# anneouyang/OuterSPACE

Measured on AMD Instinct MI355X. Metric: spgemm_output_nnz_per_s, higher is better.
Workload: dtype f64

## Files before the change

### outerspace_amd/csrc/osp_pipeline.h

```cpp
#pragma once

#define OSP_WITH_RA(ctx_, ...)                                               \
    do {                                                                     \
        if ((ctx_)->rank_atomic) { constexpr bool RA = true; __VA_ARGS__; }  \
        else { constexpr bool RA = false; __VA_ARGS__; }                     \
    } while (0)

template <class T> struct PanelWork {
    uint64_t r0, r1;
    bool whole;
    uint64_t base, count;
    Part<T> *stage;
    const uint32_t *cells = nullptr; Part<T> *qstage = nullptr;
    const HubArgs *hub = nullptr;
    bool compact = false;
    bool has_long = true;
    bool desc_only = false;
    bool walk_all = false;
};
template <class T> struct Producer {
    virtual ~Producer() {}
    virtual void produce(const PanelWork<T> &w, PhaseTimer &tm) = 0;
};

// ... 204 lines not shown
        fprintf(stderr, "[osp]   panel rows [%llu,%llu): %u tiles, %u long rows with %llu partial products -> %llu segments; direct: %llu rows, %llu "
                        "partial products, %llu cells\n",
                (unsigned long long)r0, (unsigned long long)r1, pl.p0.ntiles, nlong, (unsigned long long)pl.nh, (unsigned long long)pl.nvirt,
                (unsigned long long)pl.mode_rows[kModeDirect], (unsigned long long)pl.mode_partials[kModeDirect], (unsigned long long)ndcell);
    pl.ghist = sc.get<uint32_t>(pl.ncell + 1);
    pl.ghist_tmp = sc.get<uint32_t>(scan_scratch_entries(pl.ncell + 1));
    pl.vrow_off = sc.get<uint64_t>(pl.nvirt + 1);
    pl.vfirst = sc.get<uint8_t>(pl.nvirt + 1);
    pl.vcol0 = sc.get<uint32_t>(pl.nvirt + 1);
    pl.vcol1 = sc.get<uint32_t>(pl.nvirt + 1);
    if (pl.mode_rows[kModeDirect]) {
        pl.cells = sc.get<uint32_t>(ndcell);
        GatherPlan gp{};
        RunDesc<T> *runs = nullptr;
        const uint64_t max_runs = env.gather_max_runs.or_(0xffffffffull);
        if (ds->gather && nrund && nrd < max_runs) {
            runs = sc.get<RunDesc<T>>(std::max<uint64_t>(nrd, 1));
            pl.vrun_off = sc.get<uint32_t>(pl.nvirt + 1);
            pl.vrun_end = sc.get<uint32_t>(pl.nvirt + 1);
            gp.rdbase = rdbase; gp.vrun_off = pl.vrun_off; gp.vrun_end = pl.vrun_end;
            gp.rowruns = sc.get<uint32_t>(nlong);
            pl.nwritten = gp.nwritten = sc.get<uint32_t>(1);
            fill_async(s, {{pl.vrun_off, (pl.nvirt + 1) * sizeof(uint32_t), kNoRuns}, {gp.rowruns, (uint64_t)nlong * sizeof(uint32_t), kNoRuns},
                           {pl.nwritten, sizeof(uint32_t), 0u}});
            gp.over = env.gather_over.on;
            gp.av_in_order = ds->av_in_order ? 1u : 0u;
            pl.may_write = !gp.over;
            pl.ga.runs = runs; pl.ga.b_colidx = ds->b_colidx; pl.ga.b_vals = (const T *)ds->b_vals;
        }
        if (!(runs && gp.over) || (hub_b && pl.nblocks)) ds->ensure_chunk_off(s);
        gp.mark_skipped = ds->chunk_off_ready ? 1u : 0u;
        const bool plan_small = runs != nullptr && gp.over && nsmall != 0;
        const bool plan_big = !plan_small || nsmall < pl.mode_rows[kModeDirect];
        if (plan_small) gp.small = hsmall;
        if (ctx->env.verbose)
            fprintf(stderr, "[osp]   small planner: %llu of %llu direct rows (at most %u chunks, %u cells)\n", (unsigned long long)(plan_small ? nsmall : 0),
                    (unsigned long long)pl.mode_rows[kModeDirect], small_lim.chunks, small_lim.cells);
        tm.begin(PH_PLAN_K, s);
        if (plan_small)
            direct_plan_small_kernel<T><<<nlong, kWave, direct_plan_small_lds(small_lim.cells), s>>>(
                pl.p0.long_rows, nlong, pl.hbits, nseg, pl.vbase, pl.hoff, colbits, kCap, ds->rowfirst, ds->off, ds->bs, ds->perm, ds->b_colidx,
                pl.vrow_off, pl.vcol0, pl.vcol1, ds->chunk_off, gp, (const T *)ds->a_vals, runs);
        if (!plan_big) {  }
        else if (nlong <= 4u * ctx->cus)
            direct_plan_kernel<T, kDirectCellsBig><<<nlong, kDirectThreads, 0, s>>>(pl.p0.long_rows, nlong, pl.hmode, pl.hbits, nseg, pl.vbase, pl.hoff,
                                                                                 pl.cellbase, row_off, colbits, kCap, ds->rowfirst, ds->off, ds->bs, ds->perm,
                                                                                 ds->b_colidx, pl.vrow_off, pl.vcol0, pl.vcol1, pl.cells, ds->chunk_off, gp,
                                                                                 (const T *)ds->a_vals, runs);
        else
        direct_plan_kernel<T><<<nlong, kDirectThreads, 0, s>>>(pl.p0.long_rows, nlong, pl.hmode, pl.hbits, nseg, pl.vbase, pl.hoff, pl.cellbase, row_off,
                                                              colbits, kCap, ds->rowfirst, ds->off, ds->bs, ds->perm, ds->b_colidx, pl.vrow_off,
                                                              pl.vcol0, pl.vcol1, pl.cells, ds->chunk_off, gp, (const T *)ds->a_vals, runs);
        tm.end(PH_PLAN_K);
        if (gp.rowruns && ds->gstat) gather_stats_kernel<<<std::min(grid_for(nlong, 256), 64u), 256, 0, s>>>(pl.p0.long_rows, nlong, row_off, gp.rowruns, ds->gstat);
#ifdef OSP_PLAN_PROF
        if (ctx->env.verbose) {
            unsigned long long hp[8] = {0}, z[8] = {0};
            OSP_HIP(hipStreamSynchronize(s));
// ... 714 lines not shown
```

### outerspace_amd/csrc/osp_settings.h

```cpp
#pragma once
#include <cstdint>
#include <cstdlib>
#include <string>

namespace osp {

struct Flag {
    bool set = false;
    int value = 0;
    explicit operator bool() const { return set; }
    void parse(const char *v) { set = v != nullptr; value = v ? atoi(v) : 0; }
};
struct Switch {
    bool on = true;
    explicit operator bool() const { return on; }
    void parse(const char *v) { on = !(v && *v && atoi(v) == 0); }
};
template <class T> struct Opt {
    bool set = false;
    T value{};
    T or_(T dflt) const { return set ? value : dflt; }
};
struct Int : Opt<int> { void parse(const char *v) { if ((set = v && *v)) value = atoi(v); } };
struct Long : Opt<long> { void parse(const char *v) { if ((set = v && *v)) value = atol(v); } };
// ... 3 lines not shown
    std::string text;
    bool is(const char *w) const { return text == w; }
    void parse(const char *v) { text = v ? v : ""; }
};

enum When { PerCall, PerContext, PerProcess };

#define OSP_SETTINGS(X)                                                   \
    X(verbose, "OSP_VERBOSE", Flag, PerCall)                              \
    X(sync, "OSP_SYNC", Flag, PerProcess)                                 \
    X(poison, "OSP_POISON", Flag, PerProcess)                             \
    X(guard, "OSP_GUARD", Flag, PerProcess)                               \
    X(direct, "OSP_DIRECT", Switch, PerCall)                              \
    X(hub, "OSP_HUB", Switch, PerCall)                                    \
    X(plan_small, "OSP_PLAN_SMALL", Switch, PerCall)                      \
    X(gather_over, "OSP_GATHER_OVER", Switch, PerCall)                    \
    X(expand_rows, "OSP_EXPAND_ROWS", Switch, PerCall)                    \
    X(plan_overlap, "OSP_PLAN_OVERLAP", Switch, PerCall)                  \
    X(gather, "OSP_GATHER", Int, PerCall)                                 \
    X(split_from_b, "OSP_SPLIT_FROM_B", Int, PerCall)                     \
    X(dense_seg, "OSP_DENSE_SEG", Int, PerCall)                           \
    X(multi_subpanels, "OSP_MULTI_SUBPANELS", Int, PerCall)               \
    X(parse_threads, "OSP_PARSE_THREADS", Int, PerCall)                   \
    X(plan_small_cells, "OSP_PLAN_SMALL_CELLS", Long, PerCall)            \
    X(plan_small_chunks, "OSP_PLAN_SMALL_CHUNKS", Long, PerCall)          \
    X(direct_min_nnz, "OSP_DIRECT_MIN_NNZ", U64, PerCall)                 \
    X(direct_max, "OSP_DIRECT_MAX", U64, PerCall)                         \
    X(split_row_max, "OSP_SPLIT_ROW_MAX", U64, PerCall)                   \
    X(gather_max_runs, "OSP_GATHER_MAX_RUNS", U64, PerCall)               \
    X(bigtile_cap, "OSP_BIGTILE_CAP", U64, PerCall)                       \
    X(compact_min_waste, "OSP_COMPACT_MIN_WASTE", U64, PerCall)           \
    X(masked_heavy_min, "OSP_MASKED_HEAVY_MIN", U64, PerCall)             \
    X(masked_bucket, "OSP_MASKED_BUCKET", U64, PerCall)                   \
    X(mcl_long_min, "OSP_MCL_LONG_MIN", U64, PerCall)                     \
    X(mxm_short_cap, "OSP_MXM_SHORT_CAP", U64, PerCall)                   \
    X(mxm_batch, "OSP_MXM_BATCH", U64, PerCall)                           \
    X(mxv_group, "OSP_MXV_GROUP", U64, PerCall)                           \
    X(hub_min_share, "OSP_HUB_MIN_SHARE", Real, PerCall)                  \
    X(hub_min_run, "OSP_HUB_MIN_RUN", Real, PerCall)                      \
    X(rank, "OSP_RANK", Word, PerContext)                                 \
// ... 30 lines not shown
```

### outerspace_amd/csrc/osp_split.h

```cpp
#pragma once
#include "osp_kernels.h"

namespace osp {

#ifndef OSP_SPLIT_THREADS
#define OSP_SPLIT_THREADS 256
#endif
constexpr int kSplitThreads = OSP_SPLIT_THREADS;
#ifndef OSP_SPLIT_ROW_THREADS
#define OSP_SPLIT_ROW_THREADS 1024
#endif
#ifndef OSP_SPLIT_ROW_PRE
#define OSP_SPLIT_ROW_PRE 1
#endif
constexpr int kSplitRowThreads = OSP_SPLIT_ROW_THREADS;
#ifndef OSP_SPLIT_ROW_STRETCH
#define OSP_SPLIT_ROW_STRETCH 4096
#endif
constexpr int kSplitRowStretch = OSP_SPLIT_ROW_STRETCH;
#ifndef OSP_SPLIT_STRETCH
#define OSP_SPLIT_STRETCH 4096
#endif
constexpr int kSplitStretch = OSP_SPLIT_STRETCH;
#ifndef OSP_SPLIT_JOB_ROUNDS
// ... 553 lines not shown
    uint32_t *nwritten = nullptr;
    uint32_t over = 1;
    uint32_t mark_skipped = 1;
    uint32_t av_in_order = 0;
    const uint8_t *small = nullptr;
};
__global__ void gather_stats_kernel(const uint32_t *rows, uint32_t nlong, const uint64_t *row_off, const uint32_t *rowruns, unsigned long long *gstat) {
    uint64_t nr = 0, np = 0, nd = 0;
    for (uint32_t h = blockIdx.x * blockDim.x + threadIdx.x; h < nlong; h += gridDim.x * blockDim.x) {
        const uint32_t r = rowruns[h];
        if (r != kNoRuns) { nr++; nd += r; np += row_off[rows[h] + 1] - row_off[rows[h]]; }
    }
    nr = wave_reduce_sum<uint64_t>(nr); np = wave_reduce_sum<uint64_t>(np); nd = wave_reduce_sum<uint64_t>(nd);
    if (lane_id() == 0 && nr) { atomicAdd(&gstat[0], (unsigned long long)nr); atomicAdd(&gstat[1], (unsigned long long)np); atomicAdd(&gstat[2], (unsigned long long)nd); }
}
constexpr int kDirectCellsBig = 8 * OSP_DIRECT_CELLS_LDS;
template <class V, int CL = OSP_DIRECT_CELLS_LDS>
__global__ __launch_bounds__(kDirectThreads, (CL > OSP_DIRECT_CELLS_LDS ? 2 : 8)) void direct_plan_kernel(
    const uint32_t *__restrict__ rows, uint32_t nlong, const uint8_t *__restrict__ hmode, const uint8_t *__restrict__ hbits,
    const uint32_t *__restrict__ nseg, const uint64_t *__restrict__ vbase, const uint64_t *__restrict__ hoff,
    const uint64_t *__restrict__ cellbase, const uint64_t *__restrict__ row_off, int colbits, uint32_t cap,
    const uint32_t *__restrict__ rowfirst, const uint64_t *__restrict__ ct_off, const uint32_t *__restrict__ ct_bs,
    const uint32_t *__restrict__ perm, const uint32_t *__restrict__ b_colidx, uint64_t *__restrict__ vrow_off,
    uint32_t *__restrict__ vcol0, uint32_t *__restrict__ vcol1, uint32_t *__restrict__ cells, uint64_t *__restrict__ chunk_off,
    const GatherPlan gp, const V *__restrict__ a_vals, RunDesc<V> *__restrict__ runs) {
    constexpr int NT = kDirectThreads, NFINE = 1 << kDirectFineBits, CBL = kDirectChunkBlock, UNR = OSP_DIRECT_UNR;
    constexpr int kCellsLds = CL;
    constexpr bool kBigCells = CL > OSP_DIRECT_CELLS_LDS;
    __shared__ V avs_own[kBigCells ? CBL : 1];
    __shared__ alignas(8) uint32_t hist[NFINE + 1];
    __shared__ alignas(4) uint16_t nxt[NFINE];
    __shared__ uint8_t lut[NFINE];
    __shared__ uint32_t rbin0[kDirectMaxRanges + 2], roff[kDirectMaxRanges + 2], cursor[kDirectMaxRanges + 1];
    __shared__ uint32_t cbs[CBL], cst[CBL + 1];
    __shared__ uint32_t cellm[kCellsLds], lsm[kCellsLds];
    __shared__ uint32_t psum[NT];
    __shared__ uint32_t scratch[NT / kWave + 1];
    __shared__ uint32_t s_T, s_over;
    const uint32_t h = blockIdx.x;
    if (h >= nlong || hmode[h] != kModeDirect) return;
    if (gp.small != nullptr && gp.small[h]) return;
    OSP_PLAN_DECL
    const unsigned tid = threadIdx.x, lane = lane_id(), w = tid >> 6;
    const uint64_t above = lanes_above_mask();
    const uint32_t i = rows[h];
    const uint32_t c0 = rowfirst[i], nc = rowfirst[i + 1] - c0;
    const uint32_t b = hbits[h], nfine = 1u << b, Ta = nseg[h];
    const int sh = colbits - (int)b;
    const uint32_t q0 = (uint32_t)hoff[h];
    uint32_t *__restrict__ rb = cells + cellbase[h];
    const uint32_t lutw = (nfine + 3) / 4;
    auto load_block = [&](uint32_t cb, uint32_t nb) {
        uint32_t len[CBL / NT], bsv[CBL / NT], sum = 0;
#pragma unroll
        for (int q = 0; q < CBL / NT; q++) {
            const uint32_t j = tid * (CBL / NT) + q;
            len[q] = 0; bsv[q] = 0;
            if (j < nb) {
                const uint32_t c = c0 + cb + j;
                bsv[q] = ct_bs[c];
                len[q] = (uint32_t)(ct_off[c + 1] - ct_off[c]);
            }
            sum += len[q];
        }
        uint32_t total;
        uint32_t ex = block_excl_scan<uint32_t, NT>(sum, scratch, &total);
#pragma unroll
        for (int q = 0; q < CBL / NT; q++) {
            const uint32_t j = tid * (CBL / NT) + q;
            if (j < nb) { cst[j] = ex; cbs[j] = bsv[q] - ex; }
            ex += len[q];
        }
        if (tid == 0) cst[nb] = total;
        __syncthreads();
        return total;
    };
// ... 4 lines not shown
#pragma unroll
            for (int u = 0; u < UNR; u++) {
                const uint32_t e = base + u * kWave + lane;
                const bool valid = e < E;
                while (valid && e >= cst[c + 1]) c++;
                cu[u] = c;
                col[u] = b_colidx[valid ? cbs[c] + e : 0u];
            }
#pragma unroll
            for (int u = 0; u < UNR; u++) f(cu[u], col[u], base + u * kWave + lane < E);
        }
    };
    for (uint32_t d = tid; d <= nfine; d += NT) hist[d] = 0;
    __syncthreads();
    OSP_PLAN_MARK(0);
    uint32_t have_cb = 0, have_nb = 0, have_E = 0;
    for (uint32_t cb = 0; cb < nc; cb += CBL) {
        const uint32_t nb = min((uint32_t)CBL, nc - cb);
        const uint32_t E = load_block(cb, nb);
        OSP_PLAN_MARK(1);
        have_cb = cb; have_nb = nb; have_E = E;
        for_entries(nb, E, [&](uint32_t, uint32_t col, bool valid) {
#if OSP_PLAN_RUNS
            const uint32_t bin = valid ? col >> sh : 0xffffffffu;
            uint32_t runlen;
            if (wave_run_head(bin, valid, runlen, above)) atomicAdd(&hist[bin], runlen);
#else
            if (valid) atomicAdd(&hist[col >> sh], 1u);
#endif
        });
        __syncthreads();
        OSP_PLAN_MARK(2);
    }
    {
        constexpr int PER = NFINE / NT;
        static_assert(NFINE % NT == 0 && PER >= 1, "the fine bins are scanned PER per thread");
        uint32_t v[PER], sum = 0;
#pragma unroll
        for (int q = 0; q < PER; q++) { const uint32_t d = tid * PER + q; v[q] = d < nfine ? hist[d] : 0u; sum += v[q]; }
        uint32_t total;
        uint32_t ex = block_excl_scan<uint32_t, NT>(sum, scratch, &total);
#pragma unroll
        for (int q = 0; q < PER; q++) { const uint32_t d = tid * PER + q; if (d < nfine) hist[d] = ex; ex += v[q]; }
        if (tid == 0) hist[nfine] = total;
    }
    __syncthreads();
    for (uint32_t d = tid; d < nfine; d += NT) {
        const uint32_t lim = hist[d] + cap;
// ... 32 lines not shown
        const bool multi = nc > CB;
        V *avs = kBigCells ? avs_own : reinterpret_cast<V *>(hist);
        uint32_t *nzc = reinterpret_cast<uint32_t *>(nxt), *ncur = rbin0;
        static_assert(sizeof(nxt) >= (kDirectMaxRanges + 1) * sizeof(uint32_t), "runs per range: where the grouping's chain was");
        const uint32_t rowbase = (uint32_t)gp.rdbase[h];
        static_assert(kDirectMaxRanges + 1 <= NT, "one range per thread");
        const uint32_t bcol_t = tid <= T ? (uint32_t)min((uint64_t)rbin0[tid] << sh, (uint64_t)0xffffffffu) : 0u;
        __syncthreads();
        if (tid <= T) { nzc[tid] = 0; ncur[tid] = 0; if (tid < T) cursor[tid] = bcol_t; }
        if (!multi) { for (uint32_t cl = tid; cl < nc; cl += NT) avs[cl] = gp.av_in_order ? a_vals[c0 + cl] : a_vals[perm[c0 + cl]]; }
        __syncthreads();
        for (uint32_t cb = 0; cb < nc; cb += CB) {
            const uint32_t nb = min(CB, nc - cb);
            for (uint32_t x = tid; x < nb * T; x += NT) cellm[x] = 0;
            uint32_t E = have_E;
            if (cb != have_cb || nb != have_nb) E = load_block(cb, nb);
            else __syncthreads();
            have_cb = cb; have_nb = nb; have_E = E;
            OSP_PLAN_MARK(1);
            if (T > 1 && (uint64_t)E >= (uint64_t)nb * (T - 1) * 8u) {
                for (uint32_t x = tid; x < nb * (T - 1); x += NT) {
                    const uint32_t cl = x / (T - 1), t = x - cl * (T - 1) + 1;
                    const uint32_t col = cursor[t], b0 = cbs[cl] + cst[cl];
                    uint32_t lo = 0, hi = cst[cl + 1] - cst[cl];
                    while (lo < hi) { const uint32_t mid = (lo + hi) >> 1; if (b_colidx[b0 + mid] < col) lo = mid + 1; else hi = mid; }
                    lsm[cl * T + t] = lo;
                }
                for (uint32_t cl = tid; cl < nb; cl += NT) lsm[cl * T] = 0;
                __syncthreads();
                for (uint32_t x = tid; x < nb * T; x += NT) {
                    const uint32_t cl = x / T, t = x - cl * T;
// ... 3 lines not shown
                for_entries(nb, E, [&](uint32_t cl, uint32_t col, bool valid) {
                    const uint32_t key = valid ? __umul24(cl, T) + (uint32_t)lut[col >> sh] : 0xffffffffu;
                    uint32_t runlen;
                    if (wave_run_head(key, valid, runlen, above)) atomicAdd(&cellm[key], runlen);
                });
            }
            __syncthreads();
            OSP_PLAN_MARK(4);
            for (uint32_t x = tid; x < nb * T; x += NT) {
                const uint32_t c = cellm[x], cl = x / T, t = x - cl * T;
                if (c) atomicAdd(&nzc[t], 1u);
                if (multi) rb[lutw + (uint64_t)(cb + cl) * Ta + t] = c;
            }
            __syncthreads();
        }
        {
            const uint32_t v = tid < T ? nzc[tid] : 0u;
            uint32_t total;
            const uint32_t ex = block_excl_scan<uint32_t, NT>(v, scratch, &total);
            if (tid < T) nzc[tid] = ex;
            if (tid == 0) {
                nzc[T] = total;
                gp.rowruns[h] = total;
            }
            if (tid < T) cursor[tid] = 0;
        }
        __syncthreads();
        for (uint32_t t = tid; t < Ta; t += NT) {
            const uint64_t v = vbase[h] + t;
            gp.vrun_off[v] = rowbase + nzc[min(t, T)];
            gp.vrun_end[v] = rowbase + nzc[min(t + 1, T)];
        }
        const uint32_t G = max(1u, min((uint32_t)NT / T, 16u));
        for (uint32_t cb = 0; cb < nc; cb += CB) {
            const uint32_t nb = min(CB, nc - cb);
            if (multi) {
                if (cb != have_cb || nb != have_nb) { have_E = load_block(cb, nb); have_cb = cb; have_nb = nb; }
                for (uint32_t x = tid; x < nb * T; x += NT) { const uint32_t cl = x / T, t = x - cl * T; cellm[x] = rb[lutw + (uint64_t)(cb + cl) * Ta + t]; }
            }
            if (multi) { for (uint32_t cl = tid; cl < nb; cl += NT) avs[cl] = gp.av_in_order ? a_vals[c0 + cb + cl] : a_vals[perm[c0 + cb + cl]]; }
            __syncthreads();
            for (uint32_t cl = tid; cl < nb; cl += NT) {
                uint32_t run = 0;
                for (uint32_t t = 0; t < T; t++) { lsm[cl * T + t] = run; run += cellm[cl * T + t]; }
            }
            const uint32_t S = (nb + G - 1) / G;
            for (uint32_t t0 = 0; t0 < T; t0 += NT) {
                const uint32_t Tb = min((uint32_t)NT, T - t0);
                const uint32_t g = tid / Tb, t = t0 + (tid - g * Tb);
                const bool on = g < G;
                uint32_t run0 = 0, nrun0 = 0;
                __syncthreads();
// ... 28 lines not shown
            if (gp.mark_skipped) { for (uint32_t cl = tid; cl < nb; cl += NT) chunk_off[perm[c0 + cb + cl]] = kChunkSkip; }
            __syncthreads();
            OSP_PLAN_MARK(5);
        }
        return;
    }
    for (uint32_t d = tid; d < lutw * 4; d += NT) reinterpret_cast<uint8_t *>(rb)[d] = d < nfine ? lut[d] : (uint8_t)0;
    if (tid == 0 && gp.rdbase != nullptr && gp.nwritten) atomicAdd(gp.nwritten, 1u);
    OSP_PLAN_MARK(3);
    const uint32_t CB = max(1u, min((uint32_t)CBL, (uint32_t)kCellsLds / T));
    const uint32_t G = max(1u, min((uint32_t)NT / T, 16u));
    for (uint32_t cb = 0; cb < nc; cb += CB) {
        const uint32_t nb = min(CB, nc - cb);
        for (uint32_t x = tid; x < nb * T; x += NT) cellm[x] = 0;
        uint32_t E = have_E;
        if (cb != have_cb || nb != have_nb) E = load_block(cb, nb);
        else __syncthreads();
        have_cb = cb; have_nb = nb; have_E = E;
        OSP_PLAN_MARK(1);
        for_entries(nb, E, [&](uint32_t cl, uint32_t col, bool valid) {
#if OSP_PLAN_RUNS
            const uint32_t key = valid ? __umul24(cl, T) + (uint32_t)lut[col >> sh] : 0xffffffffu;
            uint32_t runlen;
            if (wave_run_head(key, valid, runlen, above)) atomicAdd(&cellm[key], runlen);
#else
            if (valid) atomicAdd(&cellm[__umul24(cl, T) + (uint32_t)lut[col >> sh]], 1u);
#endif
        });
        __syncthreads();
        OSP_PLAN_MARK(4);
        for (uint32_t cl = tid; cl < nb; cl += NT) {
// ... 18 lines not shown
                uint32_t run = run0;
                for (uint32_t gg = 0; gg < g; gg++) run += psum[gg * Tb + (t - t0)];
                const uint32_t rbase = q0 + roff[t];
                for (uint32_t cl = g * S; cl < min(nb, (g + 1) * S); cl++) {
                    rb[lutw + (uint64_t)(cb + cl) * Ta + t] = rbase + run - lsm[cl * T + t];
                    run += cellm[cl * T + t];
                }
                if (g == G - 1) cursor[t] = run;
            }
        }
        for (uint32_t cl = tid; cl < nb; cl += NT)
            chunk_off[perm[c0 + cb + cl]] = direct_desc((uint32_t)cellbase[h], lutw + (cb + cl) * Ta, (uint32_t)sh);
        __syncthreads();
        OSP_PLAN_MARK(5);
    }
}
__device__ __forceinline__ void wave_lds_sync() {
    __builtin_amdgcn_fence(__ATOMIC_RELEASE, "wavefront");
    __builtin_amdgcn_wave_barrier();
    __builtin_amdgcn_fence(__ATOMIC_ACQUIRE, "wavefront");
}
__device__ __forceinline__ uint32_t wave_last(uint32_t v) { return (uint32_t)__builtin_amdgcn_readlane((int)v, kWave - 1); }
constexpr size_t direct_plan_small_lds(uint32_t cells) { return (size_t)cells * sizeof(uint32_t); }
template <class V>
__global__ __launch_bounds__(kWave, 8) void direct_plan_small_kernel(
    const uint32_t *__restrict__ rows, uint32_t nlong, const uint8_t *__restrict__ hbits, const uint32_t *__restrict__ nseg,
    const uint64_t *__restrict__ vbase, const uint64_t *__restrict__ hoff, int colbits, uint32_t cap,
    const uint32_t *__restrict__ rowfirst, const uint64_t *__restrict__ ct_off, const uint32_t *__restrict__ ct_bs,
    const uint32_t *__restrict__ perm, const uint32_t *__restrict__ b_colidx, uint64_t *__restrict__ vrow_off,
    uint32_t *__restrict__ vcol0, uint32_t *__restrict__ vcol1, uint64_t *__restrict__ chunk_off, const GatherPlan gp,
    const V *__restrict__ a_vals, RunDesc<V> *__restrict__ runs) {
    constexpr int NF = 1 << kSmallFineBits, UNR = OSP_DIRECT_UNR, RMAX = kSmallRanges;
    extern __shared__ uint32_t cell[];
    __shared__ alignas(8) uint32_t hist[NF + 2];
    __shared__ uint32_t psum[kWave];
    __shared__ uint32_t cbs[kWave], cst[kWave + 1];
    __shared__ uint32_t rbin0[RMAX + 1], roff[RMAX + 1], bcol[RMAX + 1], nzc[RMAX + 1];
    static_assert(sizeof(hist) >= kSmallChunks * sizeof(V), "the A values go where the histogram was");
    static_assert(kSmallChunks <= kWave && kSmallRanges <= kWave && kSmallCellsMin >= NF, "a lane per chunk, a lane per segment, the chain in the cells");
    const uint32_t h = blockIdx.x;
    if (h >= nlong || !gp.small[h]) return;
    OSP_PLAN_DECL
    const unsigned lane = lane_id();
    const uint64_t above = lanes_above_mask();
    const uint32_t i = rows[h];
    const uint32_t c0 = rowfirst[i], nc = rowfirst[i + 1] - c0;
    const uint32_t b = hbits[h], nfine = 1u << b, Ta = nseg[h];
    const int sh = colbits - (int)b;
    const uint32_t q0 = (uint32_t)hoff[h];
    uint32_t bs = 0, len = 0, pa = 0;
    if (lane < nc) {
        const uint32_t c = c0 + lane;
        bs = ct_bs[c];
        len = (uint32_t)(ct_off[c + 1] - ct_off[c]);
        pa = perm[c];
    }
    const V av = lane < nc ? (gp.av_in_order ? a_vals[c0 + lane] : a_vals[pa]) : V(0);
    const uint32_t cincl = wave_incl_scan(len), E = wave_last(cincl);
    cst[lane] = cincl - len;
    cbs[lane] = bs - (cincl - len);
    if (lane == kWave - 1) cst[kWave] = E;
    for (uint32_t d = lane; d <= nfine; d += kWave) hist[d] = 0;
    wave_lds_sync();
    OSP_PLAN_SMALL_MARK(0);
    {
        uint32_t c = 0;
        for (uint32_t base = 0; base < E; base += UNR * kWave) {
            uint32_t col[UNR];
#pragma unroll
            for (int u = 0; u < UNR; u++) {
                const uint32_t e = base + u * kWave + lane;
// ... 1 lines not shown
                while (valid && e >= cst[c + 1]) c++;
                col[u] = b_colidx[valid ? cbs[c] + e : 0u];
            }
#pragma unroll
            for (int u = 0; u < UNR; u++) {
                if (base + u * kWave >= E) break;
                const bool valid = base + u * kWave + lane < E;
                const uint32_t bin = valid ? col[u] >> sh : 0xffffffffu;
                uint32_t runlen;
                if (wave_run_head(bin, valid, runlen, above)) atomicAdd(&hist[bin], runlen);
            }
        }
    }
    wave_lds_sync();
    OSP_PLAN_SMALL_MARK(1);
    {
        constexpr int PER = NF / kWave;
        uint32_t v[PER], sum = 0;
#pragma unroll
        for (int q = 0; q < PER; q++) { const uint32_t d = lane * PER + q; v[q] = d < nfine ? hist[d] : 0u; sum += v[q]; }
        const uint32_t incl = wave_incl_scan(sum), total = wave_last(incl);
        uint32_t ex = incl - sum;
#pragma unroll
        for (int q = 0; q < PER; q++) { const uint32_t d = lane * PER + q; if (d < nfine) hist[d] = ex; ex += v[q]; }
        if (lane == 0) hist[nfine] = total;
    }
    wave_lds_sync();
    uint32_t *nxt = cell;
    for (uint32_t d = lane; d < nfine; d += kWave) {
        const uint32_t lim = hist[d] + cap;
// ... 23 lines not shown
    if (lane < nc) avs[lane] = av;
    OSP_PLAN_SMALL_MARK(2);
    static_assert(16 * kSmallChunks <= TileCap<V>::value, "small rows never take the walk");
    const uint32_t TS = T + 1;
    wave_lds_sync();
    for (uint32_t x = lane; x < nc * (T - 1); x += kWave) {
        const uint32_t cl = x / (T - 1), t = x - cl * (T - 1) + 1;
        const uint32_t col = bcol[t], b0 = cbs[cl] + cst[cl];
        uint32_t lo = 0, hi = cst[cl + 1] - cst[cl];
        while (lo < hi) { const uint32_t mid = (lo + hi) >> 1; if (b_colidx[b0 + mid] < col) lo = mid + 1; else hi = mid; }
        cell[cl * TS + t] = lo;
    }
    if (lane < nc) { cell[lane * TS] = 0; cell[lane * TS + T] = len; }
    wave_lds_sync();
    OSP_PLAN_SMALL_MARK(3);
    const uint32_t G = max(1u, min((uint32_t)kWave / T, 16u)), S = (nc + G - 1) / G;
    const uint32_t g = lane / T, t = lane - g * T;
    const bool on = g < G;
    const uint32_t cl0 = min(nc, g * S), cl1 = min(nc, (g + 1) * S);
    {
        uint32_t sum = 0, nz = 0;
        if (on)
            for (uint32_t cl = cl0; cl < cl1; cl++) { const uint32_t c = cell[cl * TS + t + 1] - cell[cl * TS + t]; sum += c; nz += c != 0; }
        psum[lane] = sum | (nz << 21);
    }
    wave_lds_sync();
    uint32_t run = 0, nrun = 0, nzt = 0;
    if (on)
        for (uint32_t gg = 0; gg < G; gg++) {
            const uint32_t p = psum[gg * T + t];
// ... 18 lines not shown
        RunDesc<V> *__restrict__ out = runs + rowbase + nzc[t];
        for (uint32_t cl = cl0; cl < cl1; cl++) {
            const uint32_t s0 = cell[cl * TS + t], c = cell[cl * TS + t + 1] - s0;
            if (c) {
                RunDesc<V> rd;
                rd.dst = rbase + run;
                rd.src = cbs[cl] + cst[cl] + s0;
                rd.av = avs[cl];
                out[nrun++] = rd;
            }
            run += c;
        }
    }
    if (gp.mark_skipped && lane < nc) chunk_off[pa] = kChunkSkip;
    OSP_PLAN_SMALL_MARK(4);
}
__global__ void hub_rowstart_kernel(const int64_t *b_rowptr, uint64_t K, uint8_t *rowstart) {
    const uint64_t k = (uint64_t)blockIdx.x * blockDim.x + threadIdx.x;
    if (k < K && b_rowptr[k + 1] > b_rowptr[k]) rowstart[b_rowptr[k]] = 1;
}
struct HubRunFlag {
    const uint8_t *rowstart;
    const uint32_t *col;
    int sh;
    __device__ uint32_t operator()(uint64_t e) const { return (rowstart[e] || (col[e] >> sh) != (col[e - 1] >> sh)) ? 1u : 0u; }
};
__global__ void hub_runstart_end_kernel(const uint32_t *nruns_p, uint32_t *runstart, uint32_t nnz) { runstart[*nruns_p] = nnz; }
__global__ void hub_runblk_kernel(const uint32_t *__restrict__ nruns_p, const uint32_t *__restrict__ runstart, const uint32_t *__restrict__ b_colidx,
                                  int sh, uint16_t *__restrict__ runblk) {
    const uint32_t nruns = *nruns_p;
// ... 100 lines not shown
```

Baseline: 69.45 billion.

## Add persistent planner kernels with atomic row tickets and next-row prefetch

Adds persistent versions of the direct and small planner kernels, enabled by default through the OSP_PLAN_PERSIST switch. Instead of launching one block per long row, a grid capped by CU count pulls batches of rows through an atomic ticket counter. Each block prefetches the next row's header, bounds and chunk metadata while it finishes the current row. The goal is to cut launch and scheduling cost for rows that early-exit and to hide global load latency, at the price of more register pressure, ticket atomics and extra code complexity.

```diff
diff --git a/outerspace_amd/csrc/osp_pipeline.h b/outerspace_amd/csrc/osp_pipeline.h
--- a/outerspace_amd/csrc/osp_pipeline.h
+++ b/outerspace_amd/csrc/osp_pipeline.h
@@ -242,6 +242,9 @@
         GatherPlan gp{};
         RunDesc<T> *runs = nullptr;
         const uint64_t max_runs = env.gather_max_runs.or_(0xffffffffull);
+        const bool persist = env.plan_persist.on;
+        uint32_t *tickets = persist ? sc.get<uint32_t>(2 * kTicketStride) : nullptr;
+        const size_t ticket_bytes = persist ? 2 * kTicketStride * sizeof(uint32_t) : 0;
         if (ds->gather && nrund && nrd < max_runs) {
             runs = sc.get<RunDesc<T>>(std::max<uint64_t>(nrd, 1));
             pl.vrun_off = sc.get<uint32_t>(pl.nvirt + 1);
@@ -250,11 +253,13 @@
             gp.rowruns = sc.get<uint32_t>(nlong);
             pl.nwritten = gp.nwritten = sc.get<uint32_t>(1);
             fill_async(s, {{pl.vrun_off, (pl.nvirt + 1) * sizeof(uint32_t), kNoRuns}, {gp.rowruns, (uint64_t)nlong * sizeof(uint32_t), kNoRuns},
-                           {pl.nwritten, sizeof(uint32_t), 0u}});
+                           {pl.nwritten, sizeof(uint32_t), 0u}, {tickets, ticket_bytes, 0u}});
             gp.over = env.gather_over.on;
             gp.av_in_order = ds->av_in_order ? 1u : 0u;
             pl.may_write = !gp.over;
             pl.ga.runs = runs; pl.ga.b_colidx = ds->b_colidx; pl.ga.b_vals = (const T *)ds->b_vals;
+        } else {
+            zero_async(s, {{tickets, ticket_bytes}});
         }
         if (!(runs && gp.over) || (hub_b && pl.nblocks)) ds->ensure_chunk_off(s);
         gp.mark_skipped = ds->chunk_off_ready ? 1u : 0u;
@@ -264,12 +269,27 @@
         if (ctx->env.verbose)
             fprintf(stderr, "[osp]   small planner: %llu of %llu direct rows (at most %u chunks, %u cells)\n", (unsigned long long)(plan_small ? nsmall : 0),
                     (unsigned long long)pl.mode_rows[kModeDirect], small_lim.chunks, small_lim.cells);
+        const uint64_t nbig = pl.mode_rows[kModeDirect] - (plan_small ? nsmall : 0);
+        const uint64_t grid_cap = (uint64_t)std::clamp<long>(env.plan_grid.or_(0x7fffffffL), 1L, 0x7fffffffL);
+        auto plan_grid = [&](uint64_t nrows, unsigned per_cu) { return (unsigned)std::max<uint64_t>(1, std::min({nrows, (uint64_t)ctx->cus * per_cu, grid_cap})); };
         tm.begin(PH_PLAN_K, s);
-        if (plan_small)
+        if (plan_small && persist)
+            direct_plan_small_persist_kernel<T><<<plan_grid(nsmall, 32), kWave, direct_plan_small_lds(small_lim.cells), s>>>(
+                pl.p0.long_rows, nlong, pl.hbits, nseg, pl.vbase, pl.hoff, colbits, kCap, ds->rowfirst, ds->off, ds->bs, ds->perm, ds->b_colidx,
+                pl.vrow_off, pl.vcol0, pl.vcol1, ds->chunk_off, gp, (const T *)ds->a_vals, runs, tickets + kTicketStride);
+        else if (plan_small)
             direct_plan_small_kernel<T><<<nlong, kWave, direct_plan_small_lds(small_lim.cells), s>>>(
                 pl.p0.long_rows, nlong, pl.hbits, nseg, pl.vbase, pl.hoff, colbits, kCap, ds->rowfirst, ds->off, ds->bs, ds->perm, ds->b_colidx,
                 pl.vrow_off, pl.vcol0, pl.vcol1, ds->chunk_off, gp, (const T *)ds->a_vals, runs);
         if (!plan_big) {  }
+        else if (persist && nlong <= 4u * ctx->cus)
+            direct_plan_persist_kernel<T, kDirectCellsBig><<<plan_grid(nbig, 2), kDirectThreads, 0, s>>>(
+                pl.p0.long_rows, nlong, pl.hmode, pl.hbits, nseg, pl.vbase, pl.hoff, pl.cellbase, colbits, kCap, ds->rowfirst, ds->off, ds->bs, ds->perm,
+                ds->b_colidx, pl.vrow_off, pl.vcol0, pl.vcol1, pl.cells, ds->chunk_off, gp, (const T *)ds->a_vals, runs, tickets);
+        else if (persist)
+            direct_plan_persist_kernel<T><<<plan_grid(nbig, 8), kDirectThreads, 0, s>>>(
+                pl.p0.long_rows, nlong, pl.hmode, pl.hbits, nseg, pl.vbase, pl.hoff, pl.cellbase, colbits, kCap, ds->rowfirst, ds->off, ds->bs, ds->perm,
+                ds->b_colidx, pl.vrow_off, pl.vcol0, pl.vcol1, pl.cells, ds->chunk_off, gp, (const T *)ds->a_vals, runs, tickets);
         else if (nlong <= 4u * ctx->cus)
             direct_plan_kernel<T, kDirectCellsBig><<<nlong, kDirectThreads, 0, s>>>(pl.p0.long_rows, nlong, pl.hmode, pl.hbits, nseg, pl.vbase, pl.hoff,
                                                                                  pl.cellbase, row_off, colbits, kCap, ds->rowfirst, ds->off, ds->bs, ds->perm,
diff --git a/outerspace_amd/csrc/osp_settings.h b/outerspace_amd/csrc/osp_settings.h
--- a/outerspace_amd/csrc/osp_settings.h
+++ b/outerspace_amd/csrc/osp_settings.h
@@ -41,6 +41,7 @@
     X(direct, "OSP_DIRECT", Switch, PerCall)                              \
     X(hub, "OSP_HUB", Switch, PerCall)                                    \
     X(plan_small, "OSP_PLAN_SMALL", Switch, PerCall)                      \
+    X(plan_persist, "OSP_PLAN_PERSIST", Switch, PerCall)                  \
     X(gather_over, "OSP_GATHER_OVER", Switch, PerCall)                    \
     X(expand_rows, "OSP_EXPAND_ROWS", Switch, PerCall)                    \
     X(plan_overlap, "OSP_PLAN_OVERLAP", Switch, PerCall)                  \
@@ -51,6 +52,7 @@
     X(parse_threads, "OSP_PARSE_THREADS", Int, PerCall)                   \
     X(plan_small_cells, "OSP_PLAN_SMALL_CELLS", Long, PerCall)            \
     X(plan_small_chunks, "OSP_PLAN_SMALL_CHUNKS", Long, PerCall)          \
+    X(plan_grid, "OSP_PLAN_GRID", Long, PerCall)                          \
     X(direct_min_nnz, "OSP_DIRECT_MIN_NNZ", U64, PerCall)                 \
     X(direct_max, "OSP_DIRECT_MAX", U64, PerCall)                         \
     X(split_row_max, "OSP_SPLIT_ROW_MAX", U64, PerCall)                   \
diff --git a/outerspace_amd/csrc/osp_split.h b/outerspace_amd/csrc/osp_split.h
--- a/outerspace_amd/csrc/osp_split.h
+++ b/outerspace_amd/csrc/osp_split.h
@@ -591,16 +591,72 @@
     nr = wave_reduce_sum<uint64_t>(nr); np = wave_reduce_sum<uint64_t>(np); nd = wave_reduce_sum<uint64_t>(nd);
     if (lane_id() == 0 && nr) { atomicAdd(&gstat[0], (unsigned long long)nr); atomicAdd(&gstat[1], (unsigned long long)np); atomicAdd(&gstat[2], (unsigned long long)nd); }
 }
+#ifndef OSP_PLAN_AHEAD
+#define OSP_PLAN_AHEAD 3
+#endif
+#ifndef OSP_PLAN_AHEAD_SMALL
+#define OSP_PLAN_AHEAD_SMALL 2
+#endif
+constexpr uint32_t kPlanBlockRows = 32, kPlanSmallBlockRows = 64;
+constexpr uint32_t kPlanNoRow = 0xffffffffu;
+static_assert(kPlanBlockRows <= (uint32_t)kWave && kPlanSmallBlockRows <= (uint32_t)kWave, "a block's rows are a ballot");
+__device__ __forceinline__ uint32_t wave_uniform(uint32_t v) { return (uint32_t)__builtin_amdgcn_readfirstlane((int)v); }
+template <uint32_t ROWS, class F>
+__device__ __forceinline__ void plan_take_block(uint32_t *ticket, uint32_t nlong, F mine, uint32_t &base, uint64_t &mask) {
+    const unsigned lane = lane_id();
+    for (;;) {
+        uint32_t t = 0;
+        if (lane == 0) t = atomicAdd(ticket, 1u);
+        const uint64_t first = (uint64_t)wave_uniform(t) * ROWS;
+        if (first >= nlong) { base = kPlanNoRow; mask = 0; return; }
+        const uint32_t hh = (uint32_t)first + lane;
+        const uint64_t m = __builtin_amdgcn_ballot_w64(lane < ROWS && hh < nlong && mine(hh));
+        if (m) { base = (uint32_t)first; mask = m; return; }
+    }
+}
+template <int Q>
+struct PlanAhead {
+    uint32_t i = 0, c0 = 0, c1 = 0, pa = 0;
+    uint32_t bs[Q], o0[Q], o1[Q];
+    __device__ __forceinline__ void header(uint32_t hn, const uint32_t *__restrict__ rows) {
+        uint32_t hc = hn == kPlanNoRow ? 0u : hn;
+        asm("" : "+v"(hc));
+        i = rows[hc];
+    }
+    __device__ __forceinline__ void bounds(const uint32_t *__restrict__ rowfirst) { c0 = rowfirst[i]; c1 = rowfirst[i + 1]; }
+    __device__ __forceinline__ void chunks(unsigned t, uint32_t limit, const uint64_t *__restrict__ ct_off, const uint32_t *__restrict__ ct_bs,
+                                           const uint32_t *__restrict__ perm = nullptr) {
+        const uint32_t n = min(limit, c1 - c0);
+        const uint32_t *__restrict__ off32 = reinterpret_cast<const uint32_t *>(ct_off);
+#pragma unroll
+        for (int q = 0; q < Q; q++) {
+            const uint32_t j = t * Q + q;
+            const uint64_t c = j < n ? c0 + j : 0u;
+            if (ct_bs) bs[q] = ct_bs[c];
+            o0[q] = off32[2 * c];
+            o1[q] = off32[2 * c + 2];
+            if (perm) pa = perm[c];
+        }
+    }
+    __device__ __forceinline__ void all(uint32_t hn, unsigned t, uint32_t limit, const uint32_t *__restrict__ rows,
+                                        const uint32_t *__restrict__ rowfirst, const uint64_t *__restrict__ ct_off, const uint32_t *__restrict__ ct_bs,
+                                        const uint32_t *__restrict__ perm = nullptr) {
+        header(hn, rows);
+        bounds(rowfirst);
+        chunks(t, limit, ct_off, ct_bs, perm);
+    }
+};
 constexpr int kDirectCellsBig = 8 * OSP_DIRECT_CELLS_LDS;
-template <class V, int CL = OSP_DIRECT_CELLS_LDS>
-__global__ __launch_bounds__(kDirectThreads, (CL > OSP_DIRECT_CELLS_LDS ? 2 : 8)) void direct_plan_kernel(
-    const uint32_t *__restrict__ rows, uint32_t nlong, const uint8_t *__restrict__ hmode, const uint8_t *__restrict__ hbits,
+template <class V, int CL, bool PERSIST, class NextRow>
+__device__ __forceinline__ void direct_plan_row(
+    const uint32_t h, PlanAhead<kDirectChunkBlock / kDirectThreads> &ah, NextRow next_row,
+    const uint32_t *__restrict__ rows, const uint8_t *__restrict__ hbits,
     const uint32_t *__restrict__ nseg, const uint64_t *__restrict__ vbase, const uint64_t *__restrict__ hoff,
-    const uint64_t *__restrict__ cellbase, const uint64_t *__restrict__ row_off, int colbits, uint32_t cap,
+    const uint64_t *__restrict__ cellbase, int colbits, uint32_t cap,
     const uint32_t *__restrict__ rowfirst, const uint64_t *__restrict__ ct_off, const uint32_t *__restrict__ ct_bs,
     const uint32_t *__restrict__ perm, const uint32_t *__restrict__ b_colidx, uint64_t *__restrict__ vrow_off,
     uint32_t *__restrict__ vcol0, uint32_t *__restrict__ vcol1, uint32_t *__restrict__ cells, uint64_t *__restrict__ chunk_off,
-    const GatherPlan gp, const V *__restrict__ a_vals, RunDesc<V> *__restrict__ runs) {
+    const GatherPlan &gp, const V *__restrict__ a_vals, RunDesc<V> *__restrict__ runs) {
     constexpr int NT = kDirectThreads, NFINE = 1 << kDirectFineBits, CBL = kDirectChunkBlock, UNR = OSP_DIRECT_UNR;
     constexpr int kCellsLds = CL;
     constexpr bool kBigCells = CL > OSP_DIRECT_CELLS_LDS;
@@ -614,29 +670,44 @@
     __shared__ uint32_t psum[NT];
     __shared__ uint32_t scratch[NT / kWave + 1];
     __shared__ uint32_t s_T, s_over;
-    const uint32_t h = blockIdx.x;
-    if (h >= nlong || hmode[h] != kModeDirect) return;
-    if (gp.small != nullptr && gp.small[h]) return;
     OSP_PLAN_DECL
     const unsigned tid = threadIdx.x, lane = lane_id(), w = tid >> 6;
     const uint64_t above = lanes_above_mask();
-    const uint32_t i = rows[h];
-    const uint32_t c0 = rowfirst[i], nc = rowfirst[i + 1] - c0;
-    const uint32_t b = hbits[h], nfine = 1u << b, Ta = nseg[h];
+    uint32_t c0, nc, b;
+    constexpr int AH = PERSIST ? OSP_PLAN_AHEAD : 0;
+    uint32_t ah_bs[CBL / NT] = {}, ah_len[CBL / NT] = {};
+    if constexpr (AH >= 1) {
+        c0 = wave_uniform(ah.c0); nc = wave_uniform(ah.c1) - c0;
+#pragma unroll
+        for (int q = 0; q < CBL / NT; q++) {
+            if constexpr (AH >= 3) ah_bs[q] = ah.bs[q];
+            if constexpr (AH >= 2) ah_len[q] = ah.o1[q] - ah.o0[q];
+        }
+    } else {
+        const uint32_t i = rows[h];
+        c0 = rowfirst[i]; nc = rowfirst[i + 1] - c0;
+    }
+    b = hbits[h];
+    const uint32_t nfine = 1u << b, Ta = nseg[h];
     const int sh = colbits - (int)b;
     const uint32_t q0 = (uint32_t)hoff[h];
     uint32_t *__restrict__ rb = cells + cellbase[h];
     const uint32_t lutw = (nfine + 3) / 4;
-    auto load_block = [&](uint32_t cb, uint32_t nb) {
+    auto load_block = [&](uint32_t cb, uint32_t nb, auto ahead) {
         uint32_t len[CBL / NT], bsv[CBL / NT], sum = 0;
 #pragma unroll
         for (int q = 0; q < CBL / NT; q++) {
             const uint32_t j = tid * (CBL / NT) + q;
             len[q] = 0; bsv[q] = 0;
             if (j < nb) {
-                const uint32_t c = c0 + cb + j;
-                bsv[q] = ct_bs[c];
-                len[q] = (uint32_t)(ct_off[c + 1] - ct_off[c]);
+                if constexpr (decltype(ahead)::value) {
+                    bsv[q] = AH >= 3 ? ah_bs[q] : ct_bs[c0 + cb + j];
+                    len[q] = ah_len[q];
+                } else {
+                    const uint32_t c = c0 + cb + j;
+                    bsv[q] = ct_bs[c];
+                    len[q] = (uint32_t)(ct_off[c + 1] - ct_off[c]);
+                }
             }
             sum += len[q];
         }
@@ -671,10 +742,12 @@
     for (uint32_t d = tid; d <= nfine; d += NT) hist[d] = 0;
     __syncthreads();
     OSP_PLAN_MARK(0);
+    if constexpr (AH >= 1) ah.header(next_row(), rows);
     uint32_t have_cb = 0, have_nb = 0, have_E = 0;
+    const uint32_t E0 = load_block(0, min((uint32_t)CBL, nc), std::integral_constant<bool, AH >= 2>{});
     for (uint32_t cb = 0; cb < nc; cb += CBL) {
         const uint32_t nb = min((uint32_t)CBL, nc - cb);
-        const uint32_t E = load_block(cb, nb);
+        const uint32_t E = cb ? load_block(cb, nb, std::false_type{}) : E0;
         OSP_PLAN_MARK(1);
         have_cb = cb; have_nb = nb; have_E = E;
         for_entries(nb, E, [&](uint32_t, uint32_t col, bool valid) {
@@ -689,6 +762,7 @@
         __syncthreads();
         OSP_PLAN_MARK(2);
     }
+    if constexpr (AH >= 1) ah.bounds(rowfirst);
     {
         constexpr int PER = NFINE / NT;
         static_assert(NFINE % NT == 0 && PER >= 1, "the fine bins are scanned PER per thread");
@@ -751,7 +825,7 @@
             const uint32_t nb = min(CB, nc - cb);
             for (uint32_t x = tid; x < nb * T; x += NT) cellm[x] = 0;
             uint32_t E = have_E;
-            if (cb != have_cb || nb != have_nb) E = load_block(cb, nb);
+            if (cb != have_cb || nb != have_nb) E = load_block(cb, nb, std::false_type{});
             else __syncthreads();
             have_cb = cb; have_nb = nb; have_E = E;
             OSP_PLAN_MARK(1);
@@ -785,6 +859,7 @@
             }
             __syncthreads();
         }
+        if constexpr (AH >= 2) ah.chunks(tid, CBL, ct_off, AH >= 3 ? ct_bs : nullptr);
         {
             const uint32_t v = tid < T ? nzc[tid] : 0u;
             uint32_t total;
@@ -806,7 +881,7 @@
         for (uint32_t cb = 0; cb < nc; cb += CB) {
             const uint32_t nb = min(CB, nc - cb);
             if (multi) {
-                if (cb != have_cb || nb != have_nb) { have_E = load_block(cb, nb); have_cb = cb; have_nb = nb; }
+                if (cb != have_cb || nb != have_nb) { have_E = load_block(cb, nb, std::false_type{}); have_cb = cb; have_nb = nb; }
                 for (uint32_t x = tid; x < nb * T; x += NT) { const uint32_t cl = x / T, t = x - cl * T; cellm[x] = rb[lutw + (uint64_t)(cb + cl) * Ta + t]; }
             }
             if (multi) { for (uint32_t cl = tid; cl < nb; cl += NT) avs[cl] = gp.av_in_order ? a_vals[c0 + cb + cl] : a_vals[perm[c0 + cb + cl]]; }
@@ -865,7 +940,7 @@
         const uint32_t nb = min(CB, nc - cb);
         for (uint32_t x = tid; x < nb * T; x += NT) cellm[x] = 0;
         uint32_t E = have_E;
-        if (cb != have_cb || nb != have_nb) E = load_block(cb, nb);
+        if (cb != have_cb || nb != have_nb) E = load_block(cb, nb, std::false_type{});
         else __syncthreads();
         have_cb = cb; have_nb = nb; have_E = E;
         OSP_PLAN_MARK(1);
@@ -914,6 +989,69 @@
         __syncthreads();
         OSP_PLAN_MARK(5);
     }
+    if constexpr (AH >= 2) ah.chunks(tid, CBL, ct_off, AH >= 3 ? ct_bs : nullptr);
+}
+template <class V, int CL = OSP_DIRECT_CELLS_LDS>
+__global__ __launch_bounds__(kDirectThreads, (CL > OSP_DIRECT_CELLS_LDS ? 2 : 8)) void direct_plan_kernel(
+    const uint32_t *__restrict__ rows, uint32_t nlong, const uint8_t *__restrict__ hmode, const uint8_t *__restrict__ hbits,
+    const uint32_t *__restrict__ nseg, const uint64_t *__restrict__ vbase, const uint64_t *__restrict__ hoff,
+    const uint64_t *__restrict__ cellbase, const uint64_t *__restrict__ row_off, int colbits, uint32_t cap,
+    const uint32_t *__restrict__ rowfirst, const uint64_t *__restrict__ ct_off, const uint32_t *__restrict__ ct_bs,
+    const uint32_t *__restrict__ perm, const uint32_t *__restrict__ b_colidx, uint64_t *__restrict__ vrow_off,
+    uint32_t *__restrict__ vcol0, uint32_t *__restrict__ vcol1, uint32_t *__restrict__ cells, uint64_t *__restrict__ chunk_off,
+    const GatherPlan gp, const V *__restrict__ a_vals, RunDesc<V> *__restrict__ runs) {
+    const uint32_t h = blockIdx.x;
+    if (h >= nlong || hmode[h] != kModeDirect) return;
+    if (gp.small != nullptr && gp.small[h]) return;
+    PlanAhead<kDirectChunkBlock / kDirectThreads> ah;
+    direct_plan_row<V, CL, false>(h, ah, [] { return kPlanNoRow; }, rows, hbits, nseg, vbase, hoff, cellbase, colbits, cap, rowfirst, ct_off, ct_bs, perm,
+                                  b_colidx, vrow_off, vcol0, vcol1, cells, chunk_off, gp, a_vals, runs);
+}
+template <class V, int CL = OSP_DIRECT_CELLS_LDS>
+__global__ __launch_bounds__(kDirectThreads, (CL > OSP_DIRECT_CELLS_LDS ? 2 : 8)) void direct_plan_persist_kernel(
+    const uint32_t *__restrict__ rows, uint32_t nlong, const uint8_t *__restrict__ hmode, const uint8_t *__restrict__ hbits,
+    const uint32_t *__restrict__ nseg, const uint64_t *__restrict__ vbase, const uint64_t *__restrict__ hoff,
+    const uint64_t *__restrict__ cellbase, int colbits, uint32_t cap,
+    const uint32_t *__restrict__ rowfirst, const uint64_t *__restrict__ ct_off, const uint32_t *__restrict__ ct_bs,
+    const uint32_t *__restrict__ perm, const uint32_t *__restrict__ b_colidx, uint64_t *__restrict__ vrow_off,
+    uint32_t *__restrict__ vcol0, uint32_t *__restrict__ vcol1, uint32_t *__restrict__ cells, uint64_t *__restrict__ chunk_off,
+    const GatherPlan gp, const V *__restrict__ a_vals, RunDesc<V> *__restrict__ runs, uint32_t *__restrict__ ticket) {
+    constexpr int Q = kDirectChunkBlock / kDirectThreads;
+    __shared__ uint32_t s_base[2], s_mask[2];
+    static_assert(kPlanBlockRows <= 32, "a block's rows in one word");
+    const unsigned tid = threadIdx.x, w = tid >> 6;
+    auto take = [&](uint32_t set) {
+        uint32_t base;
+        uint64_t mask;
+        plan_take_block<kPlanBlockRows>(ticket, nlong, [&](uint32_t hh) { return hmode[hh] == kModeDirect && !(gp.small != nullptr && gp.small[hh]); }, base, mask);
+        if (tid == 0) { s_base[set] = base; s_mask[set] = (uint32_t)mask; }
+    };
+    if (w == 0) take(0);
+    __syncthreads();
+    uint32_t set = 0, base = wave_uniform(s_base[0]), mask = wave_uniform(s_mask[0]);
+    if (base == kPlanNoRow) return;
+    PlanAhead<Q> ah;
+    if (OSP_PLAN_AHEAD >= 1) ah.all(base + (uint32_t)__builtin_ctz(mask), tid, kDirectChunkBlock, rows, rowfirst, ct_off, OSP_PLAN_AHEAD >= 3 ? ct_bs : nullptr);
+    for (;;) {
+        const uint32_t h = base + (uint32_t)__builtin_ctz(mask);
+        mask &= mask - 1;
+        if (mask == 0 && w == 0) take(set ^ 1);
+        direct_plan_row<V, CL, true>(
+            h, ah,
+            [&]() -> uint32_t {
+                if (mask) return base + (uint32_t)__builtin_ctz(mask);
+                const uint32_t nb = wave_uniform(s_base[set ^ 1]);
+                return nb == kPlanNoRow ? kPlanNoRow : nb + (uint32_t)__builtin_ctz(wave_uniform(s_mask[set ^ 1]));
+            },
+            rows, hbits, nseg, vbase, hoff, cellbase, colbits, cap, rowfirst, ct_off, ct_bs, perm, b_colidx, vrow_off, vcol0, vcol1, cells, chunk_off,
+            gp, a_vals, runs);
+        __syncthreads();
+        if (mask == 0) {
+            set ^= 1;
+            base = wave_uniform(s_base[set]); mask = wave_uniform(s_mask[set]);
+            if (base == kPlanNoRow) break;
+        }
+    }
 }
 __device__ __forceinline__ void wave_lds_sync() {
     __builtin_amdgcn_fence(__ATOMIC_RELEASE, "wavefront");
@@ -922,13 +1060,14 @@
 }
 __device__ __forceinline__ uint32_t wave_last(uint32_t v) { return (uint32_t)__builtin_amdgcn_readlane((int)v, kWave - 1); }
 constexpr size_t direct_plan_small_lds(uint32_t cells) { return (size_t)cells * sizeof(uint32_t); }
-template <class V>
-__global__ __launch_bounds__(kWave, 8) void direct_plan_small_kernel(
-    const uint32_t *__restrict__ rows, uint32_t nlong, const uint8_t *__restrict__ hbits, const uint32_t *__restrict__ nseg,
+template <class V, bool PERSIST>
+__device__ __forceinline__ void direct_plan_small_row(
+    const uint32_t h, PlanAhead<1> &ah, const uint32_t hn,
+    const uint32_t *__restrict__ rows, const uint8_t *__restrict__ hbits, const uint32_t *__restrict__ nseg,
     const uint64_t *__restrict__ vbase, const uint64_t *__restrict__ hoff, int colbits, uint32_t cap,
     const uint32_t *__restrict__ rowfirst, const uint64_t *__restrict__ ct_off, const uint32_t *__restrict__ ct_bs,
     const uint32_t *__restrict__ perm, const uint32_t *__restrict__ b_colidx, uint64_t *__restrict__ vrow_off,
-    uint32_t *__restrict__ vcol0, uint32_t *__restrict__ vcol1, uint64_t *__restrict__ chunk_off, const GatherPlan gp,
+    uint32_t *__restrict__ vcol0, uint32_t *__restrict__ vcol1, uint64_t *__restrict__ chunk_off, const GatherPlan &gp,
     const V *__restrict__ a_vals, RunDesc<V> *__restrict__ runs) {
     constexpr int NF = 1 << kSmallFineBits, UNR = OSP_DIRECT_UNR, RMAX = kSmallRanges;
     extern __shared__ uint32_t cell[];
@@ -938,23 +1077,33 @@
     __shared__ uint32_t rbin0[RMAX + 1], roff[RMAX + 1], bcol[RMAX + 1], nzc[RMAX + 1];
     static_assert(sizeof(hist) >= kSmallChunks * sizeof(V), "the A values go where the histogram was");
     static_assert(kSmallChunks <= kWave && kSmallRanges <= kWave && kSmallCellsMin >= NF, "a lane per chunk, a lane per segment, the chain in the cells");
-    const uint32_t h = blockIdx.x;
-    if (h >= nlong || !gp.small[h]) return;
     OSP_PLAN_DECL
     const unsigned lane = lane_id();
     const uint64_t above = lanes_above_mask();
-    const uint32_t i = rows[h];
-    const uint32_t c0 = rowfirst[i], nc = rowfirst[i + 1] - c0;
-    const uint32_t b = hbits[h], nfine = 1u << b, Ta = nseg[h];
+    uint32_t c0, nc, b;
+    uint32_t bs = 0, len = 0, pa = 0;
+    constexpr int AH = PERSIST ? OSP_PLAN_AHEAD_SMALL : 0;
+    if constexpr (AH >= 1) {
+        c0 = wave_uniform(ah.c0); nc = wave_uniform(ah.c1) - c0;
+        ah.header(hn, rows);
+    } else {
+        const uint32_t i = rows[h];
+        c0 = rowfirst[i]; nc = rowfirst[i + 1] - c0;
+    }
+    b = hbits[h];
+    if constexpr (AH >= 2) {
+        if (lane < nc) { bs = ah.bs[0]; len = ah.o1[0] - ah.o0[0]; pa = ah.pa; }
+    } else {
+        if (lane < nc) {
+            const uint32_t c = c0 + lane;
+            bs = ct_bs[c];
+            len = (uint32_t)(ct_off[c + 1] - ct_off[c]);
+            pa = perm[c];
+        }
+    }
+    const uint32_t nfine = 1u << b, Ta = nseg[h];
     const int sh = colbits - (int)b;
     const uint32_t q0 = (uint32_t)hoff[h];
-    uint32_t bs = 0, len = 0, pa = 0;
-    if (lane < nc) {
-        const uint32_t c = c0 + lane;
-        bs = ct_bs[c];
-        len = (uint32_t)(ct_off[c + 1] - ct_off[c]);
-        pa = perm[c];
-    }
     const V av = lane < nc ? (gp.av_in_order ? a_vals[c0 + lane] : a_vals[pa]) : V(0);
     const uint32_t cincl = wave_incl_scan(len), E = wave_last(cincl);
     cst[lane] = cincl - len;
@@ -986,6 +1135,7 @@
     }
     wave_lds_sync();
     OSP_PLAN_SMALL_MARK(1);
+    if constexpr (AH >= 1) ah.bounds(rowfirst);
     {
         constexpr int PER = NF / kWave;
         uint32_t v[PER], sum = 0;
@@ -1039,6 +1189,7 @@
     if (lane < nc) { cell[lane * TS] = 0; cell[lane * TS + T] = len; }
     wave_lds_sync();
     OSP_PLAN_SMALL_MARK(3);
+    if constexpr (AH >= 2) ah.chunks(lane, (uint32_t)kWave, ct_off, ct_bs, perm);
     const uint32_t G = max(1u, min((uint32_t)kWave / T, 16u)), S = (nc + G - 1) / G;
     const uint32_t g = lane / T, t = lane - g * T;
     const bool on = g < G;
@@ -1087,6 +1238,47 @@
     }
     if (gp.mark_skipped && lane < nc) chunk_off[pa] = kChunkSkip;
     OSP_PLAN_SMALL_MARK(4);
+}
+template <class V>
+__global__ __launch_bounds__(kWave, 8) void direct_plan_small_kernel(
+    const uint32_t *__restrict__ rows, uint32_t nlong, const uint8_t *__restrict__ hbits, const uint32_t *__restrict__ nseg,
+    const uint64_t *__restrict__ vbase, const uint64_t *__restrict__ hoff, int colbits, uint32_t cap,
+    const uint32_t *__restrict__ rowfirst, const uint64_t *__restrict__ ct_off, const uint32_t *__restrict__ ct_bs,
+    const uint32_t *__restrict__ perm, const uint32_t *__restrict__ b_colidx, uint64_t *__restrict__ vrow_off,
+    uint32_t *__restrict__ vcol0, uint32_t *__restrict__ vcol1, uint64_t *__restrict__ chunk_off, const GatherPlan gp,
+    const V *__restrict__ a_vals, RunDesc<V> *__restrict__ runs) {
+    const uint32_t h = blockIdx.x;
+    if (h >= nlong || !gp.small[h]) return;
+    PlanAhead<1> ah;
+    direct_plan_small_row<V, false>(h, ah, kPlanNoRow, rows, hbits, nseg, vbase, hoff, colbits, cap, rowfirst, ct_off, ct_bs, perm, b_colidx, vrow_off, vcol0,
+                                    vcol1, chunk_off, gp, a_vals, runs);
+}
+template <class V>
+__global__ __launch_bounds__(kWave, 8) void direct_plan_small_persist_kernel(
+    const uint32_t *__restrict__ rows, uint32_t nlong, const uint8_t *__restrict__ hbits, const uint32_t *__restrict__ nseg,
+    const uint64_t *__restrict__ vbase, const uint64_t *__restrict__ hoff, int colbits, uint32_t cap,
+    const uint32_t *__restrict__ rowfirst, const uint64_t *__restrict__ ct_off, const uint32_t *__restrict__ ct_bs,
+    const uint32_t *__restrict__ perm, const uint32_t *__restrict__ b_colidx, uint64_t *__restrict__ vrow_off,
+    uint32_t *__restrict__ vcol0, uint32_t *__restrict__ vcol1, uint64_t *__restrict__ chunk_off, const GatherPlan gp,
+    const V *__restrict__ a_vals, RunDesc<V> *__restrict__ runs, uint32_t *__restrict__ ticket) {
+    const unsigned lane = lane_id();
+    auto mine = [&](uint32_t hh) { return gp.small[hh] != 0; };
+    uint32_t base;
+    uint64_t mask;
+    plan_take_block<kPlanSmallBlockRows>(ticket, nlong, mine, base, mask);
+    if (base == kPlanNoRow) return;
+    PlanAhead<1> ah;
+    if (OSP_PLAN_AHEAD_SMALL >= 1) ah.all(base + (uint32_t)__builtin_ctzll(mask), lane, (uint32_t)kWave, rows, rowfirst, ct_off, ct_bs, perm);
+    for (;;) {
+        const uint32_t h = base + (uint32_t)__builtin_ctzll(mask);
+        mask &= mask - 1;
+        if (mask == 0) plan_take_block<kPlanSmallBlockRows>(ticket, nlong, mine, base, mask);
+        const uint32_t hn = base == kPlanNoRow ? kPlanNoRow : base + (uint32_t)__builtin_ctzll(mask);
+        direct_plan_small_row<V, true>(h, ah, hn, rows, hbits, nseg, vbase, hoff, colbits, cap, rowfirst, ct_off, ct_bs, perm, b_colidx, vrow_off, vcol0, vcol1,
+                                       chunk_off, gp, a_vals, runs);
+        if (hn == kPlanNoRow) break;
+        wave_lds_sync();
+    }
 }
 __global__ void hub_rowstart_kernel(const int64_t *b_rowptr, uint64_t K, uint8_t *rowstart) {
     const uint64_t k = (uint64_t)blockIdx.x * blockDim.x + threadIdx.x;
```

Result: slower. 61.00 billion (-12.2%).
